# saidwivedi/TokenHMR

Hardware: NVIDIA H100
Metric: images/sec (256x192) at bs=64 per GPU, full TokenHMR forward (higher is better)
Workload: dtype f16 operands / f32 accumulate

## Files before the change

tokenhmr_b200/csrc/gemm_host.cuh:

```cuda
#pragma once
#include "common.cuh"

#include "gemm_wgmma.cuh"

namespace thmr {

struct GemmPlan {
  CUtensorMap tmA, tmB;
  GemmParams p;
  int bn;
  int grid;
  int cluster;
  int fp8;
  int epi;
};

struct GemmDesc {
  const __half* A; int lda; long long a_rows;
  const __half* B; int ldb;
  int M, N, K;
  const float* bias = nullptr;
  const float* resid = nullptr; int ldr = 0; int resid_mod = 0;
  int act = kActNone; int act32 = 0;
  float* out32 = nullptr; int ld32 = 0;
  __half* out16 = nullptr; int ld16 = 0;
  int taps = 1; int cin = 0; int tap_row0 = 0; int tap_stride = 0;
  int seq_pitch = 0, seq_lo = 0, seq_hi = 0;
  float alpha = 1.0f;
  long long* argmin_out = nullptr; const float* row_sq = nullptr; const float* col_sq = nullptr;
  int* screen_rows = nullptr; int* screen_count = nullptr; const float* screen_cmax2 = nullptr;
  float screen_rel = 0.f, screen_abs = 0.f; int screen_row0 = 0;
  const int* row_map = nullptr; const int* m_dev = nullptr; int m_dev_off = 0;
  int force_bn = 0;
  int force_epi = 0;
  unsigned long long* stamp = nullptr;
  int fp8 = 0;
  const float* a_scale = nullptr; int ld_as = 0;
  const float* w_scale = nullptr;
  uint8_t* out8 = nullptr; int ld8 = 0; float* out8_scale = nullptr; int ld8s = 0;
};

inline int pick_bn(int M, int N, int K, bool staged_epilogue, bool fast_epilogue, int force) {
  if (force) return force;
  const int sms = num_sms();
  const int tm = (M + kGemmBM - 1) / kGemmBM;
  const int num_kb = (K + kGemmBK - 1) / kGemmBK;
  int best = 256;
  double best_cost = -1;
  const int cands[4] = {256, 128, 64, 32};
  for (int i = 0; i < 4; ++i) {
    const int bn = cands[i];
    const long tiles = static_cast<long>(tm) * ((N + bn - 1) / bn);
    const long waves = (tiles + sms - 1) / sms;
    const double mma = 4.0 * bn;
    const double feed = (128.0 + bn) * 128.0 / 32.0;
    const double epilogue = !staged_epilogue                 ? 0.0
                            : fast_epilogue && bn >= 128      ? 5000.0 * bn / 128
                            : bn == 256                       ? 55000.0
                                                              : 7000.0 * bn / 128;
    const double cost = waves * (num_kb * ((mma > feed ? mma : feed) + 40.0) + epilogue);
    if (best_cost < 0 || cost < best_cost) { best_cost = cost; best = bn; }
  }
  return best;
}

inline int pick_bn_fp8(int M, int N, int K) {
  const int sms = num_sms();
  const int tm = (M + kGemmBM - 1) / kGemmBM;
  const int num_kb = (K + 127) / 128;
  int best = 128;
  double best_cost = -1;
  const int cands[2] = {128, 64};
  for (int i = 0; i < 2; ++i) {
    const int bn = cands[i];
    const long tiles = static_cast<long>(tm) * ((N + bn - 1) / bn);
    const long waves = (tiles + sms - 1) / sms;
    const double mma = 4.0 * bn;
    const double feed = (128.0 + bn) * 128.0 / 32.0;
    const double cost = waves * (num_kb * ((mma > feed ? mma : feed) + bn + 40.0) + 7000.0 * bn / 128);
    if (best_cost < 0 || cost < best_cost) { best_cost = cost; best = bn; }
  }
  return best;
}

inline int gemm_pick_epi(const GemmDesc& d, int bn, int cluster) {
  auto al16 = [](const void* q) { return (reinterpret_cast<uintptr_t>(q) & 15) == 0; };
  if ((bn != 128 && bn != 256) || cluster != 1 || d.argmin_out || d.resid_mod || d.seq_pitch || d.act32 || !al16(d.bias))
    return kEpiGeneral;
  if (d.out16 && !d.out32 && !d.resid && d.ld16 % 8 == 0 && al16(d.out16)) {
    if (d.act == kActNone) return d.bias ? kEpiBiasF16 : kEpiF16;
    if (d.act == kActGelu && d.bias) return kEpiBiasGeluF16;
  }
// ... 5 lines not shown

inline int make_tmap_2d_e4m3(CUtensorMap* out, const void* base, uint64_t rows, uint64_t cols, uint64_t ld,
                             uint32_t box_rows, uint32_t box_cols) {
  return make_tmap_2d(out, CU_TENSOR_MAP_DATA_TYPE_UINT8, 1, base, rows, cols, ld, box_rows, box_cols,
                      CU_TENSOR_MAP_SWIZZLE_128B);
}

inline int gemm_make_plan_fp8(const GemmDesc& d, GemmPlan* plan) {
  THMR_CHECK(d.M > 0 && d.N > 0 && d.K > 0 && d.K % 128 == 0, "gemm fp8: bad shape %dx%dx%d (K %% 128 != 0)", d.M, d.N,
             d.K);
  THMR_CHECK(d.out32 || d.out16 || d.out8, "gemm fp8: no output");
  THMR_CHECK(d.a_scale && d.w_scale, "gemm fp8: missing block scales");
  THMR_CHECK(!d.argmin_out && d.taps == 1 && !d.m_dev && !d.row_map, "gemm fp8: plain GEMMs only");
  const long m_pad = (d.M + kGemmBM - 1) / kGemmBM * kGemmBM;
  THMR_CHECK(d.ld_as >= m_pad && d.ld_as % 4 == 0 && (reinterpret_cast<uintptr_t>(d.a_scale) & 15) == 0,
             "gemm fp8: activation scales need a 16-byte aligned [K/128][>= %ld] layout (ld_as %d)", m_pad, d.ld_as);
  int bn = d.force_bn ? d.force_bn : d.out8 ? 128 : pick_bn_fp8(d.M, d.N, d.K);
  THMR_CHECK(bn == 64 || bn == 128, "gemm fp8: block_n %d (64 or 128)", bn);
  THMR_CHECK(!d.out8 || (bn == 128 && d.out8_scale && d.ld8s >= d.M && !d.resid && !d.act32 && !d.seq_pitch),
             "gemm fp8: e4m3 output needs block_n 128, its scale array and no residual / mask / act32");
  GemmParams& p = plan->p;
  memset(&p, 0, sizeof(p));
  p.M = d.M; p.N = d.N; p.K = d.K;
  p.out32 = d.out32; p.ld32 = d.ld32; p.out16 = d.out16; p.ld16 = d.ld16;
  p.bias = d.bias; p.resid = d.resid; p.ldr = d.ldr; p.resid_mod = d.resid_mod; p.act = d.act; p.act32 = d.act32;
  p.seq_pitch = d.seq_pitch; p.seq_lo = d.seq_lo; p.seq_hi = d.seq_hi;
  p.alpha = d.alpha;
  p.stamp = d.stamp;
  p.kblocks_per_tap = d.K / 128;
  p.a_scale = d.a_scale; p.ld_as = d.ld_as; p.w_scale = d.w_scale;
  p.out8 = d.out8; p.ld8 = d.ld8; p.out8_scale = d.out8_scale; p.ld8s = d.ld8s;
  THMR_TRY(make_tmap_2d_e4m3(&plan->tmA, d.A, d.a_rows, d.K, d.lda, kGemmBM, 128));
  THMR_TRY(make_tmap_2d_e4m3(&plan->tmB, d.B, d.N, d.K, d.ldb, bn, 128));
  THMR_CHECK(d.force_epi == 0 || d.force_epi == 1 + kEpiGeneral, "gemm fp8: general epilogue only");
  plan->bn = bn;
  plan->cluster = 1;
  plan->fp8 = 1;
  plan->epi = kEpiGeneral;
  const long tiles_m = (d.M + kGemmBM - 1) / kGemmBM;
  const long tiles = tiles_m * ((d.N + bn - 1) / bn);
  p.m_fast = (tiles_m > 1 && d.M < d.N) ? 1 : 0;
  const long slots = num_sms();
  plan->grid = static_cast<int>(tiles < slots ? tiles : slots);
  return THMR_OK;
}

inline int gemm_make_plan(const GemmDesc& d, GemmPlan* plan) {
  if (d.fp8) return gemm_make_plan_fp8(d, plan);
  THMR_CHECK(d.M > 0 && d.N > 0 && d.K > 0, "gemm: bad shape %dx%dx%d", d.M, d.N, d.K);
  THMR_CHECK(d.out32 || d.out16 || d.argmin_out, "gemm: no output");
  const int cluster = d.force_bn == 512 ? 2 : 1;
  THMR_CHECK(cluster == 1 || !d.argmin_out, "gemm: block_n 512 (CTA pair) does not support the arg-min modes");
  const bool fast_epi = gemm_pick_epi(d, 256, cluster) != kEpiGeneral;
  const int bn = cluster == 2 ? 256 : pick_bn(d.M, d.N, d.K, d.argmin_out == nullptr, fast_epi, d.force_bn);
  THMR_CHECK(bn == 32 || bn == 64 || bn == 128 || bn == 256, "gemm: bad block_n %d", bn);
  GemmParams& p = plan->p;
  memset(&p, 0, sizeof(p));
  p.M = d.M; p.N = d.N; p.K = d.K;
  p.out32 = d.out32; p.ld32 = d.ld32; p.out16 = d.out16; p.ld16 = d.ld16;
  p.bias = d.bias; p.resid = d.resid; p.ldr = d.ldr; p.resid_mod = d.resid_mod; p.act = d.act; p.act32 = d.act32;
  p.seq_pitch = d.seq_pitch; p.seq_lo = d.seq_lo; p.seq_hi = d.seq_hi;
  p.alpha = d.alpha; p.argmin_out = d.argmin_out; p.row_sq = d.row_sq; p.col_sq = d.col_sq;
  THMR_CHECK(!d.screen_rows || (d.argmin_out && d.screen_count && d.screen_cmax2),
             "gemm: screened arg-min needs its queue");
  THMR_CHECK((!d.m_dev && !d.row_map) || d.argmin_out, "gemm: device row count / row map are arg-min options");
  p.screen_rows = d.screen_rows; p.screen_count = d.screen_count; p.screen_cmax2 = d.screen_cmax2;
  p.screen_rel = d.screen_rel; p.screen_abs = d.screen_abs; p.screen_row0 = d.screen_row0;
  p.row_map = d.row_map; p.m_dev = d.m_dev; p.m_dev_off = d.m_dev_off;
  p.stamp = d.stamp;
  const int num_kb = (d.K + kGemmBK - 1) / kGemmBK;
  uint64_t a_cols = d.K;
  if (d.taps > 1) {
    THMR_CHECK(d.cin % kGemmBK == 0 && d.K == d.taps * d.cin, "gemm conv: cin %d taps %d K %d", d.cin, d.taps, d.K);
    p.kblocks_per_tap = d.cin / kGemmBK;
    p.tap_row0 = d.tap_row0; p.tap_stride = d.tap_stride;
    a_cols = d.cin;
  } else {
    p.kblocks_per_tap = num_kb;
  }
  THMR_TRY(make_tmap_2d_f16(&plan->tmA, d.A, d.a_rows, a_cols, d.lda, kGemmBM, kGemmBK, CU_TENSOR_MAP_SWIZZLE_128B));
  THMR_TRY(make_tmap_2d_f16(&plan->tmB, d.B, d.N, d.K, d.ldb, bn / cluster, kGemmBK, CU_TENSOR_MAP_SWIZZLE_128B));
  plan->bn = bn;
  plan->cluster = cluster;
  plan->fp8 = 0;
  plan->epi = gemm_pick_epi(d, bn, cluster);
  THMR_CHECK(d.force_epi == 0 || d.force_epi - 1 == kEpiGeneral || d.force_epi - 1 == plan->epi,
             "gemm: epilogue kind %d does not fit this GEMM (its kind is %d)", d.force_epi - 1, plan->epi);
  if (d.force_epi) plan->epi = d.force_epi - 1;
  const long tiles_m = (d.M + kGemmBM * cluster - 1) / (kGemmBM * cluster);
  const long tiles = d.argmin_out ? tiles_m : tiles_m * ((d.N + bn - 1) / bn);
  p.m_fast = (!d.argmin_out && tiles_m > 1 && d.M < d.N) ? 1 : 0;
  const long slots = num_sms() / cluster;
  plan->grid = cluster * static_cast<int>(tiles < slots ? tiles : slots);
  return THMR_OK;
}

template <int BN, int STAGES, int CLUSTER = 1, bool FP8 = false, int EPI = kEpiGeneral, bool TIMELINE = false>
inline int gemm_launch_t(const GemmPlan& plan, cudaStream_t stream) {
  using S = GemmSmem<BN, STAGES, FP8>;
  static_assert(S::kTotal <= 232448, "GEMM shared memory exceeds 227 KB");
  static bool configured = false;
  if (!configured) {
    THMR_CUDA(cudaFuncSetAttribute(gemm_f16_tn_kernel<BN, STAGES, CLUSTER, FP8, EPI, TIMELINE>, cudaFuncAttributeMaxDynamicSharedMemorySize,
                                   S::kTotal));
    configured = true;
  }
  cudaLaunchConfig_t cfg = {};
  cfg.gridDim = dim3(plan.grid);
  cfg.blockDim = dim3(kGemmThreads);
  cfg.dynamicSmemBytes = S::kTotal;
  cfg.stream = stream;
  cudaLaunchAttribute attr[1];
  attr[0].id = cudaLaunchAttributeClusterDimension;
  attr[0].val.clusterDim.x = CLUSTER;
  attr[0].val.clusterDim.y = 1;
  attr[0].val.clusterDim.z = 1;
  cfg.attrs = attr;
  cfg.numAttrs = 1;
  THMR_CUDA(cudaLaunchKernelEx(&cfg, gemm_f16_tn_kernel<BN, STAGES, CLUSTER, FP8, EPI, TIMELINE>, plan.tmA, plan.tmB, plan.p));
  return THMR_OK;
}

template <int BN, int STAGES, bool TIMELINE>
inline int gemm_launch_epi(const GemmPlan& plan, cudaStream_t stream) {
  switch (plan.epi) {
    case kEpiGeneral: return gemm_launch_t<BN, STAGES, 1, false, kEpiGeneral, TIMELINE>(plan, stream);
    case kEpiF16: return gemm_launch_t<BN, STAGES, 1, false, kEpiF16, TIMELINE>(plan, stream);
    case kEpiBiasF16: return gemm_launch_t<BN, STAGES, 1, false, kEpiBiasF16, TIMELINE>(plan, stream);
    case kEpiBiasGeluF16: return gemm_launch_t<BN, STAGES, 1, false, kEpiBiasGeluF16, TIMELINE>(plan, stream);
    case kEpiBiasResidF32: return gemm_launch_t<BN, STAGES, 1, false, kEpiBiasResidF32, TIMELINE>(plan, stream);
  }
  return fail(THMR_ERR_INVALID, "gemm: unsupported epilogue kind %d", plan.epi);
}

inline int gemm_launch_plain(const GemmPlan& plan, cudaStream_t stream) {
  if (plan.fp8) {
    if (plan.bn == 128) return gemm_launch_t<128, 5, 1, true>(plan, stream);
    if (plan.bn == 64) return gemm_launch_t<64, 7, 1, true>(plan, stream);
    return fail(THMR_ERR_INVALID, "gemm fp8: unsupported block_n %d", plan.bn);
  }
  if (plan.cluster == 2) return gemm_launch_t<256, 4, 2>(plan, stream);
  switch (plan.bn) {
    case 256: return gemm_launch_epi<256, 4, false>(plan, stream);
    case 128: return gemm_launch_epi<128, 6, false>(plan, stream);
    case 64: return gemm_launch_t<64, 8>(plan, stream);
    case 32: return gemm_launch_t<32, 8>(plan, stream);
  }
  return fail(THMR_ERR_INVALID, "gemm: unsupported block_n %d", plan.bn);
}

template <bool TIMELINE = false>
inline int gemm_launch(const GemmPlan& plan, cudaStream_t stream) {
// ... 13 lines not shown
```

tokenhmr_b200/csrc/gemm_wgmma.cuh:

```cuda
#pragma once
#include "common.cuh"
#include "ptx.cuh"

namespace thmr {

enum : int { kActNone = 0, kActGelu = 1, kActRelu = 2 };

enum : int { kEpiGeneral = 0, kEpiF16 = 1, kEpiBiasF16 = 2, kEpiBiasGeluF16 = 3, kEpiBiasResidF32 = 4 };

struct GemmParams {
  int M, N, K;
  float* out32;
  int ld32;
  __half* out16;
  int ld16;
  const float* bias;
  const float* resid;
  int ldr;
  int resid_mod;
  int act;
  int act32;
  int kblocks_per_tap;
  int tap_row0, tap_stride;
  int seq_pitch, seq_lo, seq_hi;
  float alpha;
  long long* argmin_out;
  const float* row_sq;
  const float* col_sq;
  int* screen_rows;
  int* screen_count;
  const float* screen_cmax2;
  float screen_rel, screen_abs;
  int screen_row0;
  const int* row_map;
  const int* m_dev;
  int m_dev_off;
  unsigned long long* stamp;
  int m_fast;
  const float* a_scale;
  int ld_as;
  const float* w_scale;
// ... 17 lines not shown
    m_blk = start;
    n_blk = 0;
  }
  __device__ bool valid() const { return m_stationary ? (m_blk < tiles_m) : (tile < num_tiles); }
  __device__ int m0(int bm) const { return (m_stationary ? m_blk : (m_fast ? tile % tiles_m : tile / tiles_n)) * bm; }
  __device__ int n0(int bn) const { return (m_stationary ? n_blk : (m_fast ? tile / tiles_m : tile % tiles_n)) * bn; }
  __device__ bool last_n() const { return n_blk == tiles_n - 1; }
  __device__ void next() {
    if (m_stationary) {
      if (++n_blk == tiles_n) { n_blk = 0; m_blk += stride; }
    } else {
      tile += stride;
    }
  }
};

constexpr int kGemmBM = 128;
constexpr int kGemmBK = 64;
constexpr int kGemmConsumerWarps = 8;
constexpr int kGemmThreads = 32 * kGemmConsumerWarps + 128;
constexpr int kWarpTma = kGemmConsumerWarps;

template <int BN>
constexpr int gemm_chunk() { return BN == 64 || BN == 128 ? 64 : 32; }

template <bool FP8>
constexpr int gemm_bk() { return FP8 ? 128 : kGemmBK; }

template <int BN, int STAGES, bool FP8 = false>
struct GemmSmem {
  static constexpr uint32_t kABytes = kGemmBM * kGemmBK * 2;
  static constexpr uint32_t kBBytes = BN * kGemmBK * 2;
  static constexpr uint32_t kStageBytes = kABytes + kBBytes;
  static constexpr uint32_t kScaleOffset = STAGES * kStageBytes;
  static constexpr uint32_t kScaleBytes = FP8 ? STAGES * kGemmBM * 4 : 0;
  static constexpr uint32_t kBarOffset = kScaleOffset + kScaleBytes;
  static constexpr uint32_t kEpiOffset = kBarOffset + 256;
  static constexpr uint32_t kEpiBytes = 2 * 64 * gemm_chunk<BN>() * 4;
  static constexpr uint32_t kRowScaleOffset = kEpiOffset + kEpiBytes;
  static constexpr uint32_t kRowScaleBytes = FP8 ? kGemmBM * 4 : 0;
  static constexpr uint32_t kTotal = kRowScaleOffset + kRowScaleBytes + 1024;
};

__device__ __forceinline__ float gelu_erf(float x) {
  const float a = fabsf(x) * 0.70710678118654752f;
  float p = fmaf(0.0000430638f, a, 0.0002765672f);
  p = fmaf(p, a, 0.0001520143f);
  p = fmaf(p, a, 0.0092705272f);
  p = fmaf(p, a, 0.0422820123f);
  p = fmaf(p, a, 0.0705230784f);
  p = fmaf(p, a, 1.0f);
  p *= p; p *= p; p *= p; p *= p;
  float r;
  asm("rcp.approx.ftz.f32 %0, %1;" : "=f"(r) : "f"(p));
  const float e = 1.0f - r;
  return fmaf(x, 0.5f, __fmul_rn(__fmul_rn(fabsf(x), 0.5f), e));
}

template <int BN>
__device__ __forceinline__ void wgmma_tile_k16(float (&acc)[BN / 2], uint64_t da, uint64_t db, uint32_t scale_d) {
  if constexpr (BN == 32) wgmma_m64n32k16(acc, da, db, scale_d);
  else if constexpr (BN == 64) wgmma_m64n64k16(acc, da, db, scale_d);
  else if constexpr (BN == 128) wgmma_m64n128k16(acc, da, db, scale_d);
  else wgmma_m64n256k16(acc, da, db, scale_d);
}

template <int BN>
__device__ __forceinline__ void wgmma_tile_k32_e4m3(float (&acc)[BN / 2], uint64_t da, uint64_t db, uint32_t scale_d) {
  if constexpr (BN == 64) wgmma_m64n64k32_e4m3(acc, da, db, scale_d);
  else wgmma_m64n128k32_e4m3(acc, da, db, scale_d);
}

// ... 132 lines not shown
          if (full && p.ld8 % 8 == 0 && (reinterpret_cast<uintptr_t>(p.out8) & 7) == 0) {
            *reinterpret_cast<uint2*>(o) = make_uint2(q[0] | (static_cast<uint32_t>(q[1]) << 16),
                                                      q[2] | (static_cast<uint32_t>(q[3]) << 16));
          } else {
#pragma unroll
            for (int e = 0; e < 8; ++e)
              if (col + e < p.N) o[e] = static_cast<uint8_t>(q[e >> 1] >> (8 * (e & 1)));
          }
        }
      }
      if (p.out16) {
        if (!p.act32 && !final_vals) {
#pragma unroll
          for (int e = 0; e < 8; ++e) v[e] = gemm_act(p.act, v[e]);
        }
        __half* o = p.out16 + static_cast<size_t>(row) * p.ld16 + col;
        if (full && vec16) {
          uint4 q;
          __half2* h2 = reinterpret_cast<__half2*>(&q);
#pragma unroll
          for (int e = 0; e < 4; ++e) h2[e] = __floats2half2_rn(v[2 * e], v[2 * e + 1]);
          *reinterpret_cast<uint4*>(o) = q;
        } else {
#pragma unroll
          for (int e = 0; e < 8; ++e)
            if (col + e < p.N) o[e] = __float2half_rn(v[e]);
        }
      }
    }
    named_barrier_sync(bar_id, 128);
  }
}

template <int EPI>
__device__ __forceinline__ void gemm_epilogue_kind_tail(const GemmParams& p, const float (&v)[8], int row, int col) {
#pragma unroll
  for (int e = 0; e < 8; ++e) {
    if (col + e >= p.N) break;
    float x = __fmul_rn(v[e], p.alpha);
    if constexpr (EPI != kEpiF16) x = __fadd_rn(x, __ldg(p.bias + col + e));
    if constexpr (EPI == kEpiBiasResidF32) {
      const size_t i = static_cast<size_t>(row) * p.ld32 + col + e;
      p.out32[i] = __fadd_rn(x, p.resid[static_cast<size_t>(row) * p.ldr + col + e]);
    } else {
      if constexpr (EPI == kEpiBiasGeluF16) x = gelu_erf(x);
      p.out16[static_cast<size_t>(row) * p.ld16 + col + e] = __float2half_rn(x);
    }
  }
}

template <int BN, int EPI>
__device__ __forceinline__ void gemm_epilogue_kind(const GemmParams& p, const float (&acc)[BN / 2], uint32_t stage,
                                                   int m0w, int n0, int M_eff, uint32_t bar_id) {
  constexpr bool kBias = EPI != kEpiF16;
  constexpr bool kResid = EPI == kEpiBiasResidF32;
  constexpr int CH = gemm_chunk<BN>();
  constexpr int OCT = CH / 8;
  constexpr int ITEMS = OCT / 2;
  const int lane = threadIdx.x & 31;
  const int w4 = (threadIdx.x >> 5) & 3;
  const int fr = w4 * 16 + (lane >> 2);
  const int fswz = (((lane >> 2) & 3) << 1) | ((lane >> 4) & 1);
  const int rswz = ((lane & 3) << 1) | ((lane >> 2) & 1);
#pragma unroll 1
  for (int c = 0; c < BN / CH; ++c) {
#pragma unroll
    for (int cc = 0; cc < BN / CH; ++cc)
      if (cc == c) gemm_stage_chunk<BN>(acc, cc, stage, fr, fswz, lane);
    named_barrier_sync(bar_id, 128);

    const int ccol = n0 + c * CH + 8 * (lane >> 3);
    float bias[ITEMS / 2][8];
    float res[ITEMS][8];
    if constexpr (kBias && !(kResid && ITEMS == 2)) {
#pragma unroll
      for (int ob = 0; ob < ITEMS / 2; ++ob) {
        const int col = ccol + 32 * ob;
        if (col + 8 <= p.N) {
          const float4 b0 = __ldg(reinterpret_cast<const float4*>(p.bias + col));
          const float4 b1 = __ldg(reinterpret_cast<const float4*>(p.bias + col + 4));
          bias[ob][0] = b0.x; bias[ob][1] = b0.y; bias[ob][2] = b0.z; bias[ob][3] = b0.w;
          bias[ob][4] = b1.x; bias[ob][5] = b1.y; bias[ob][6] = b1.z; bias[ob][7] = b1.w;
        }
      }
    }
    if constexpr (kResid) {
#pragma unroll
      for (int k = 0; k < ITEMS; ++k) {
        const int row = m0w + 8 * (w4 + 4 * (k & 1)) + (lane & 7);
        const int col = ccol + 32 * (k >> 1);
        if (row < M_eff && col + 8 <= p.N) {
          const float* r = p.resid + static_cast<size_t>(row) * p.ldr + col;
          const float4 x0 = *reinterpret_cast<const float4*>(r);
          const float4 x1 = *reinterpret_cast<const float4*>(r + 4);
          res[k][0] = x0.x; res[k][1] = x0.y; res[k][2] = x0.z; res[k][3] = x0.w;
          res[k][4] = x1.x; res[k][5] = x1.y; res[k][6] = x1.z; res[k][7] = x1.w;
        }
      }
    }
#pragma unroll
    for (int k = 0; k < ITEMS; ++k) {
      const int lr = 8 * (w4 + 4 * (k & 1)) + (lane & 7);
      const int oct = 4 * (k >> 1) + (lane >> 3);
      const int row = m0w + lr;
      const int col = ccol + 32 * (k >> 1);
      if (row >= M_eff || col >= p.N) continue;
      float v[8];
#pragma unroll
      for (int h = 0; h < 2; ++h) {
        const int u = 2 * oct + h;
        const float4 s = lds_f32x4(stage + 4 * (lr * CH + (((u & ~7) | ((u ^ rswz) & 7)) << 2)));
        v[4 * h] = s.x; v[4 * h + 1] = s.y; v[4 * h + 2] = s.z; v[4 * h + 3] = s.w;
      }
      if (col + 8 > p.N) {
        gemm_epilogue_kind_tail<EPI>(p, v, row, col);
        continue;
      }
      if constexpr (kResid && ITEMS == 2) {
        const float4 b0 = __ldg(reinterpret_cast<const float4*>(p.bias + col));
        const float4 b1 = __ldg(reinterpret_cast<const float4*>(p.bias + col + 4));
        bias[0][0] = b0.x; bias[0][1] = b0.y; bias[0][2] = b0.z; bias[0][3] = b0.w;
        bias[0][4] = b1.x; bias[0][5] = b1.y; bias[0][6] = b1.z; bias[0][7] = b1.w;
      }
#pragma unroll
      for (int e = 0; e < 8; ++e) {
        v[e] = __fmul_rn(v[e], p.alpha);
        if constexpr (kBias) v[e] = __fadd_rn(v[e], bias[k >> 1][e]);
        if constexpr (kResid) v[e] = __fadd_rn(v[e], res[k][e]);
        if constexpr (EPI == kEpiBiasGeluF16) v[e] = gelu_erf(v[e]);
      }
      if constexpr (kResid) {
        float4* o = reinterpret_cast<float4*>(p.out32 + static_cast<size_t>(row) * p.ld32 + col);
        o[0] = make_float4(v[0], v[1], v[2], v[3]);
        o[1] = make_float4(v[4], v[5], v[6], v[7]);
      } else {
        uint4 q;
        __half2* h2 = reinterpret_cast<__half2*>(&q);
#pragma unroll
        for (int e = 0; e < 4; ++e) h2[e] = __floats2half2_rn(v[2 * e], v[2 * e + 1]);
        *reinterpret_cast<uint4*>(p.out16 + static_cast<size_t>(row) * p.ld16 + col) = q;
      }
    }
    named_barrier_sync(bar_id, 128);
  }
}

template <int BN>
__device__ __forceinline__ void gemm_row_scales_e4m3(const GemmParams& p, float (&acc)[BN / 2], int m0, int n0,
                                                     int r0, int c0, int wg, int M_eff, uint32_t row_inv) {
#pragma unroll
  for (int i = 0; i < 2; ++i) {
    float amax = 0.f;
#pragma unroll
    for (int j = 0; j < BN / 8; ++j) {
#pragma unroll
      for (int c = 0; c < 2; ++c) {
        const int col = n0 + 8 * j + c0 + c;
        float v = acc[4 * j + 2 * i + c] * p.alpha;
        if (p.bias && col < p.N) v += __ldg(p.bias + col);
        v = gemm_act(p.act, v);
        acc[4 * j + 2 * i + c] = v;
        if (col < p.N) amax = fmaxf(amax, fabsf(v));
      }
    }
    amax = fmaxf(amax, __shfl_xor_sync(0xffffffffu, amax, 1));
    amax = fmaxf(amax, __shfl_xor_sync(0xffffffffu, amax, 2));
    const float s = e4m3_scale(amax);
    const int r = r0 + 8 * i;
    if ((threadIdx.x & 3) == 0) {
      sts_f32(row_inv + 4 * (r - wg * 64), 1.0f / s);
      if (m0 + r < M_eff) p.out8_scale[static_cast<size_t>(n0 / 128) * p.ld8s + m0 + r] = s;
    }
  }
}

template <int BN, int STAGES, int CLUSTER, bool FP8 = false, int EPI = kEpiGeneral, bool TIMELINE = false>
__global__ void __launch_bounds__(kGemmThreads, 1)
gemm_f16_tn_kernel(const __grid_constant__ CUtensorMap tmA, const __grid_constant__ CUtensorMap tmB, const GemmParams p) {
  using S = GemmSmem<BN, STAGES, FP8>;
  constexpr int BK = gemm_bk<FP8>();
  static_assert(BN == 32 || BN == 64 || BN == 128 || BN == 256, "BN must be a power of two in [32,256]");
  static_assert(CLUSTER == 1 || (CLUSTER == 2 && BN >= 128), "cluster pairs split B in two halves of >= 64 rows");
  static_assert(!FP8 || (CLUSTER == 1 && (BN == 64 || BN == 128)), "FP8: two accumulator sets fit at BN <= 128");
  static_assert(EPI == kEpiGeneral || (!FP8 && CLUSTER == 1 && BN >= 128), "epilogue kinds: fp16 BN 128 / 256 only");
  static_assert(!TIMELINE || (!FP8 && CLUSTER == 1), "timeline: fp16 single-CTA kernels only");

  extern __shared__ uint8_t smem_raw[];
  uint8_t* smem = reinterpret_cast<uint8_t*>((reinterpret_cast<uintptr_t>(smem_raw) + 1023) & ~uintptr_t(1023));
  uint64_t* full_bar = reinterpret_cast<uint64_t*>(smem + S::kBarOffset);
  uint64_t* empty_bar = full_bar + STAGES;

  const int warp = threadIdx.x >> 5;
  const int lane = threadIdx.x & 31;

  int M_eff = p.M;
  if (p.m_dev != nullptr) {
    const int m = __ldg(p.m_dev) - p.m_dev_off;
    M_eff = m < 0 ? 0 : (m < p.M ? m : p.M);
  }
  constexpr int kRows = kGemmBM * CLUSTER;
  const int tiles_m = (M_eff + kRows - 1) / kRows;
  const int tiles_n = (p.N + BN - 1) / BN;
  const int num_kb = (p.K + BK - 1) / BK;
  const bool m_stationary = p.argmin_out != nullptr;
  const int rank = CLUSTER == 2 ? static_cast<int>(cluster_ctarank()) : 0;
  const int tile0 = static_cast<int>(blockIdx.x) / CLUSTER, tile_step = static_cast<int>(gridDim.x) / CLUSTER;

  stamp_start(p.stamp);
  if (threadIdx.x == 0) {
    for (int s = 0; s < STAGES; ++s) {
      mbar_init(&full_bar[s], 1);
      mbar_init(&empty_bar[s], kGemmConsumerWarps * CLUSTER);
    }
    fence_mbar_init();
  }
  if (warp == kWarpTma && lane == 0) {
    tma_prefetch_desc(&tmA);
    tma_prefetch_desc(&tmB);
  }
  if constexpr (CLUSTER == 2) cluster_sync_all();
  else __syncthreads();

  if (warp >= kWarpTma) {
    asm volatile("setmaxnreg.dec.sync.aligned.u32 40;");
    if (warp == kWarpTma && lane == 0) {
      int stage = 0;
      uint32_t phase = 0;
      for (TileIter it(tiles_m, tiles_n, m_stationary, p.m_fast != 0, tile0, tile_step); it.valid(); it.next()) {
        const int m0 = it.m0(kRows) + rank * kGemmBM;
        const int n0 = it.n0(BN);
        for (int kb = 0; kb < num_kb; ++kb) {
          if constexpr (CLUSTER == 2) mbar_wait_cluster(&empty_bar[stage], phase ^ 1);
          else mbar_wait(&empty_bar[stage], phase ^ 1);
          uint8_t* sa = smem + stage * S::kStageBytes;
          uint8_t* sb = sa + S::kABytes;
          const int tap = kb / p.kblocks_per_tap;
          const int kk = kb - tap * p.kblocks_per_tap;
          mbar_arrive_expect_tx(&full_bar[stage], S::kStageBytes + (FP8 ? kGemmBM * 4 : 0));
          tma_load_2d(sa, &tmA, &full_bar[stage], kk * BK, m0 + p.tap_row0 + tap * p.tap_stride);
          if constexpr (CLUSTER == 2)
            tma_load_2d_mcast(sb + rank * (BN / 2) * 128, &tmB, &full_bar[stage], kb * BK, n0 + rank * (BN / 2), 3);
          else
            tma_load_2d(sb, &tmB, &full_bar[stage], kb * BK, n0);
          if constexpr (FP8)
            bulk_load_1d(smem + S::kScaleOffset + stage * kGemmBM * 4, p.a_scale + static_cast<size_t>(kb) * p.ld_as + m0,
                         kGemmBM * 4, &full_bar[stage]);
          if (++stage == STAGES) { stage = 0; phase ^= 1; }
        }
      }
    }
    if constexpr (CLUSTER == 2) cluster_sync_all();
    return;
  }

  asm volatile("setmaxnreg.inc.sync.aligned.u32 232;");
  const int wg = warp >> 2;
  const uint32_t smem_base = smem_u32(smem);
  const bool vec_r = p.resid && p.ldr % 4 == 0 && aligned16(p.resid);
  const bool vec32 = p.out32 && p.ld32 % 4 == 0 && aligned16(p.out32);
  const bool vec16 = p.out16 && p.ld16 % 8 == 0 && aligned16(p.out16);
  const uint32_t epi_stage = smem_base + S::kEpiOffset + wg * 64 * gemm_chunk<BN>() * 4;
  const bool screen = p.argmin_out != nullptr && p.screen_rows != nullptr;
  const float m2a = -2.0f * p.alpha;
  const int r0 = wg * 64 + (warp & 3) * 16 + (lane >> 2);
  const int c0 = 2 * (lane & 3);
  float best[2] = {INFINITY, INFINITY}, second[2] = {INFINITY, INFINITY};
  int best_idx[2] = {0, 0};
  int stage = 0;
  uint32_t phase = 0;
  float acc[BN / 2];
  float tile[FP8 ? BN / 2 : 1];

  auto release = [&](int s) {
    __syncwarp();
    if (lane == 0) {
      if constexpr (CLUSTER == 2) {
        mbar_arrive_cluster(&empty_bar[s], 0);
        mbar_arrive_cluster(&empty_bar[s], 1);
      } else {
        mbar_arrive(&empty_bar[s]);
      }
    }
  };
  auto stamp = [&](const TileIter& it, int k) {
    if (TIMELINE && p.timeline != nullptr && (threadIdx.x & 127) == 0) {
      const int slot = (it.tile - tile0) / tile_step;
      if (slot < p.timeline_slots)
        p.timeline[((static_cast<size_t>(blockIdx.x) * p.timeline_slots + slot) * 2 + wg) * 4 + k] = globaltimer();
    }
  };
  if (TIMELINE && p.timeline != nullptr && threadIdx.x == 0) p.timeline_sm[blockIdx.x] = static_cast<int>(smid());
  for (TileIter it(tiles_m, tiles_n, m_stationary, p.m_fast != 0, tile0, tile_step); it.valid(); it.next()) {
    const int m0 = it.m0(kRows) + rank * kGemmBM;
    const int n0 = it.n0(BN);
// ... 77 lines not shown
#pragma unroll
          for (int off = 1; off <= 2; off <<= 1) {
            const float ob = __shfl_xor_sync(0xffffffffu, best[i], off);
            const int oi = __shfl_xor_sync(0xffffffffu, best_idx[i], off);
            const float os = __shfl_xor_sync(0xffffffffu, second[i], off);
            second[i] = fminf(fminf(second[i], os), fmaxf(best[i], ob));
            if (ob < best[i] || (ob == best[i] && oi < best_idx[i])) { best[i] = ob; best_idx[i] = oi; }
          }
          const int row = m0 + r0 + 8 * i;
          const bool row_ok = row < M_eff;
          if ((lane & 3) == 0 && row_ok) p.argmin_out[p.row_map ? __ldg(p.row_map + row) : row] = best_idx[i];
          if (screen) {
            const float x2 = row_ok ? __ldg(p.row_sq + row) : 0.f;
            const float tau = p.screen_rel * sqrtf(x2 * cm2) + p.screen_abs * (x2 + cm2) + 1e-12f;
            const bool redo = (lane & 3) == 0 && row_ok && !(second[i] - best[i] > tau);
            const unsigned mask = __ballot_sync(0xffffffffu, redo);
            if (mask != 0u) {
              const int leader = __ffs(mask) - 1;
              int base = 0;
              if (lane == leader) base = atomicAdd(p.screen_count, __popc(mask));
              base = __shfl_sync(0xffffffffu, base, leader);
              if (redo) p.screen_rows[base + __popc(mask & ((1u << lane) - 1u))] = p.screen_row0 + row;
            }
          }
          best[i] = INFINITY;
          second[i] = INFINITY;
          best_idx[i] = 0;
        }
      }
    } else if constexpr (FP8) {
      const uint32_t row_inv = smem_base + S::kRowScaleOffset + wg * 64 * 4;
      if (p.out8) gemm_row_scales_e4m3<BN>(p, acc, m0, n0, r0, c0, wg, M_eff, row_inv);
      gemm_epilogue_rows<BN, true>(p, acc, epi_stage, m0 + wg * 64, n0, M_eff, 1 + wg, vec_r, vec32, vec16, row_inv);
    } else if constexpr (EPI != kEpiGeneral) {
      gemm_epilogue_kind<BN, EPI>(p, acc, epi_stage, m0 + wg * 64, n0, M_eff, 1 + wg);
    } else {
      gemm_epilogue_rows<BN>(p, acc, epi_stage, m0 + wg * 64, n0, M_eff, 1 + wg, vec_r, vec32, vec16);
    }
    if constexpr (TIMELINE) stamp(it, 3);
  }
  if constexpr (CLUSTER == 2) cluster_sync_all();
}

}
```

tokenhmr_b200/csrc/ptx.cuh:

```cuda
#pragma once
#include <cuda.h>
#include <cuda_fp16.h>
#include <cuda_runtime.h>
#include <stdint.h>

namespace thmr {

__device__ unsigned int g_pipeline_timeout = 0;
constexpr uint32_t kSpinLimit = 1u << 24;

__device__ __forceinline__ uint32_t smem_u32(const void* p) {
  return static_cast<uint32_t>(__cvta_generic_to_shared(p));
}

__device__ __forceinline__ void sts_f32x2(uint32_t a, float x, float y) {
  asm volatile("st.shared.v2.f32 [%0], {%1, %2};" ::"r"(a), "f"(x), "f"(y));
}
__device__ __forceinline__ float4 lds_f32x4(uint32_t a) {
  float4 v;
  asm volatile("ld.shared.v4.f32 {%0, %1, %2, %3}, [%4];" : "=f"(v.x), "=f"(v.y), "=f"(v.z), "=f"(v.w) : "r"(a));
  return v;
}
__device__ __forceinline__ void sts_f32(uint32_t a, float x) { asm volatile("st.shared.f32 [%0], %1;" ::"r"(a), "f"(x)); }
__device__ __forceinline__ float lds_f32(uint32_t a) {
  float v;
  asm volatile("ld.shared.f32 %0, [%1];" : "=f"(v) : "r"(a));
  return v;
}
__device__ __forceinline__ void named_barrier_sync(uint32_t id, uint32_t threads) {
  asm volatile("bar.sync %0, %1;" ::"r"(id), "r"(threads) : "memory");
}

__device__ __forceinline__ unsigned long long globaltimer() {
  unsigned long long t;
  asm volatile("mov.u64 %0, %%globaltimer;" : "=l"(t));
  return t;
}
__device__ __forceinline__ uint32_t smid() {
  uint32_t s;
  asm volatile("mov.u32 %0, %%smid;" : "=r"(s));
  return s;
}

__device__ __forceinline__ uint32_t lane_id() {
  uint32_t l;
  asm volatile("mov.u32 %0, %%laneid;" : "=r"(l));
  return l;
}

__device__ __forceinline__ void mbar_init(uint64_t* bar, uint32_t count) {
  asm volatile("mbarrier.init.shared::cta.b64 [%0], %1;" ::"r"(smem_u32(bar)), "r"(count) : "memory");
}
__device__ __forceinline__ void fence_mbar_init() {
  asm volatile("fence.mbarrier_init.release.cluster;" ::: "memory");
}
__device__ __forceinline__ void fence_proxy_async_smem() {
// ... 57 lines not shown
        "selp.u32 %0, 1, 0, P;\n\t"
        "}\n"
        : "=r"(ok)
        : "r"(smem_u32(bar)), "r"(parity)
        : "memory");
    if (ok) return true;
  }
  atomicExch(&g_pipeline_timeout, 1u);
  return false;
}

__device__ __forceinline__ void tma_prefetch_desc(const CUtensorMap* m) {
  asm volatile("prefetch.tensormap [%0];" ::"l"(reinterpret_cast<uint64_t>(m)) : "memory");
}
__device__ __forceinline__ void tma_load_2d(void* smem_dst, const CUtensorMap* m, uint64_t* bar, int32_t c0,
                                            int32_t c1) {
  asm volatile(
      "cp.async.bulk.tensor.2d.shared::cluster.global.mbarrier::complete_tx::bytes"
      " [%0], [%1, {%3, %4}], [%2];"
      :
      : "r"(smem_u32(smem_dst)), "l"(reinterpret_cast<uint64_t>(m)), "r"(smem_u32(bar)), "r"(c0), "r"(c1)
      : "memory");
}
__device__ __forceinline__ void tma_load_2d_mcast(void* smem_dst, const CUtensorMap* m, uint64_t* bar, int32_t c0,
                                                  int32_t c1, uint16_t cta_mask) {
  asm volatile(
      "cp.async.bulk.tensor.2d.shared::cluster.global.mbarrier::complete_tx::bytes.multicast::cluster"
      " [%0], [%1, {%3, %4}], [%2], %5;"
      :
      : "r"(smem_u32(smem_dst)), "l"(reinterpret_cast<uint64_t>(m)), "r"(smem_u32(bar)), "r"(c0), "r"(c1),
        "h"(cta_mask)
      : "memory");
}
__device__ __forceinline__ void tma_store_2d(const CUtensorMap* m, const void* smem_src, int32_t c0, int32_t c1) {
  asm volatile("cp.async.bulk.tensor.2d.global.shared::cta.bulk_group [%0, {%2, %3}], [%1];"
               :
               : "l"(reinterpret_cast<uint64_t>(m)), "r"(smem_u32(smem_src)), "r"(c0), "r"(c1)
               : "memory");
}
__device__ __forceinline__ void tma_store_commit() { asm volatile("cp.async.bulk.commit_group;" ::: "memory"); }
template <int N>
__device__ __forceinline__ void tma_store_wait_read() {
  asm volatile("cp.async.bulk.wait_group.read %0;" ::"n"(N) : "memory");
}
template <int N>
__device__ __forceinline__ void tma_store_wait() {
  asm volatile("cp.async.bulk.wait_group %0;" ::"n"(N) : "memory");
}

__device__ __forceinline__ uint64_t make_wgmma_desc_sw128(uint32_t saddr) {
  uint64_t d = 0;
  d |= static_cast<uint64_t>((saddr >> 4) & 0x3FFF);
  d |= static_cast<uint64_t>(1) << 16;
  d |= static_cast<uint64_t>(1024 >> 4) << 32;
  d |= static_cast<uint64_t>(1) << 62;
  return d;
}
__device__ __forceinline__ void wgmma_fence() { asm volatile("wgmma.fence.sync.aligned;" ::: "memory"); }
__device__ __forceinline__ void wgmma_commit() { asm volatile("wgmma.commit_group.sync.aligned;" ::: "memory"); }
template <int N>
__device__ __forceinline__ void wgmma_wait() {
  asm volatile("wgmma.wait_group.sync.aligned %0;" ::"n"(N) : "memory");
}
template <int N>
__device__ __forceinline__ void wgmma_fence_operand(float (&d)[N]) {
#pragma unroll
  for (int i = 0; i < N; ++i) asm volatile("" : "+f"(d[i])::"memory");
}

__device__ __forceinline__ void wgmma_m64n32k16(float (&d)[16], uint64_t da, uint64_t db, uint32_t scale_d) {
// ... 65 lines not shown
```

Baseline: 1690.

## Store fp16 GEMM epilogues through swizzled shared memory with TMA bulk stores

The fp16 epilogue kinds (plain, bias, bias+GELU) now convert accumulators to half, write them into a 128B-swizzled shared-memory staging block and issue asynchronous TMA 2D stores, instead of staging fp32 and having threads write global memory. A third tensor map for the output is built on the host and passed to the kernel. The residual fp32 epilogue is split into its own specialised function, and the block-N cost model now weights TMA-store and residual epilogues differently. The shared-memory layout grows each warpgroup's epilogue block to 16 KB, and the kernel waits for outstanding stores before exiting. The aim is to cut epilogue time and let stores overlap with the next tile's main loop.

```diff
diff --git a/tokenhmr_b200/csrc/gemm_host.cuh b/tokenhmr_b200/csrc/gemm_host.cuh
--- a/tokenhmr_b200/csrc/gemm_host.cuh
+++ b/tokenhmr_b200/csrc/gemm_host.cuh
@@ -7,6 +7,7 @@
 
 struct GemmPlan {
   CUtensorMap tmA, tmB;
+  CUtensorMap tmC;
   GemmParams p;
   int bn;
   int grid;
@@ -40,7 +41,7 @@
   uint8_t* out8 = nullptr; int ld8 = 0; float* out8_scale = nullptr; int ld8s = 0;
 };
 
-inline int pick_bn(int M, int N, int K, bool staged_epilogue, bool fast_epilogue, int force) {
+inline int pick_bn(int M, int N, int K, bool staged_epilogue, int epi_kind, int force) {
   if (force) return force;
   const int sms = num_sms();
   const int tm = (M + kGemmBM - 1) / kGemmBM;
@@ -54,10 +55,11 @@
     const long waves = (tiles + sms - 1) / sms;
     const double mma = 4.0 * bn;
     const double feed = (128.0 + bn) * 128.0 / 32.0;
-    const double epilogue = !staged_epilogue                 ? 0.0
-                            : fast_epilogue && bn >= 128      ? 5000.0 * bn / 128
-                            : bn == 256                       ? 55000.0
-                                                              : 7000.0 * bn / 128;
+    const double epilogue = !staged_epilogue                                 ? 0.0
+                            : bn >= 128 && gemm_epi_tma_store(epi_kind)       ? 2500.0 * bn / 128
+                            : bn >= 128 && epi_kind == kEpiBiasResidF32       ? 12000.0 * bn / 128
+                            : bn == 256                                       ? 55000.0
+                                                                              : 7000.0 * bn / 128;
     const double cost = waves * (num_kb * ((mma > feed ? mma : feed) + 40.0) + epilogue);
     if (best_cost < 0 || cost < best_cost) { best_cost = cost; best = bn; }
   }
@@ -129,6 +131,7 @@
   p.out8 = d.out8; p.ld8 = d.ld8; p.out8_scale = d.out8_scale; p.ld8s = d.ld8s;
   THMR_TRY(make_tmap_2d_e4m3(&plan->tmA, d.A, d.a_rows, d.K, d.lda, kGemmBM, 128));
   THMR_TRY(make_tmap_2d_e4m3(&plan->tmB, d.B, d.N, d.K, d.ldb, bn, 128));
+  memset(&plan->tmC, 0, sizeof(plan->tmC));
   THMR_CHECK(d.force_epi == 0 || d.force_epi == 1 + kEpiGeneral, "gemm fp8: general epilogue only");
   plan->bn = bn;
   plan->cluster = 1;
@@ -148,8 +151,8 @@
   THMR_CHECK(d.out32 || d.out16 || d.argmin_out, "gemm: no output");
   const int cluster = d.force_bn == 512 ? 2 : 1;
   THMR_CHECK(cluster == 1 || !d.argmin_out, "gemm: block_n 512 (CTA pair) does not support the arg-min modes");
-  const bool fast_epi = gemm_pick_epi(d, 256, cluster) != kEpiGeneral;
-  const int bn = cluster == 2 ? 256 : pick_bn(d.M, d.N, d.K, d.argmin_out == nullptr, fast_epi, d.force_bn);
+  const int kind = gemm_pick_epi(d, 256, cluster);
+  const int bn = cluster == 2 ? 256 : pick_bn(d.M, d.N, d.K, d.argmin_out == nullptr, kind, d.force_bn);
   THMR_CHECK(bn == 32 || bn == 64 || bn == 128 || bn == 256, "gemm: bad block_n %d", bn);
   GemmParams& p = plan->p;
   memset(&p, 0, sizeof(p));
@@ -184,6 +187,9 @@
   THMR_CHECK(d.force_epi == 0 || d.force_epi - 1 == kEpiGeneral || d.force_epi - 1 == plan->epi,
              "gemm: epilogue kind %d does not fit this GEMM (its kind is %d)", d.force_epi - 1, plan->epi);
   if (d.force_epi) plan->epi = d.force_epi - 1;
+  memset(&plan->tmC, 0, sizeof(plan->tmC));
+  if (gemm_epi_tma_store(plan->epi))
+    THMR_TRY(make_tmap_2d_f16(&plan->tmC, d.out16, d.M, d.N, d.ld16, 64, 64, CU_TENSOR_MAP_SWIZZLE_128B));
   const long tiles_m = (d.M + kGemmBM * cluster - 1) / (kGemmBM * cluster);
   const long tiles = d.argmin_out ? tiles_m : tiles_m * ((d.N + bn - 1) / bn);
   p.m_fast = (!d.argmin_out && tiles_m > 1 && d.M < d.N) ? 1 : 0;
@@ -214,7 +220,8 @@
   attr[0].val.clusterDim.z = 1;
   cfg.attrs = attr;
   cfg.numAttrs = 1;
-  THMR_CUDA(cudaLaunchKernelEx(&cfg, gemm_f16_tn_kernel<BN, STAGES, CLUSTER, FP8, EPI, TIMELINE>, plan.tmA, plan.tmB, plan.p));
+  THMR_CUDA(cudaLaunchKernelEx(&cfg, gemm_f16_tn_kernel<BN, STAGES, CLUSTER, FP8, EPI, TIMELINE>, plan.tmA, plan.tmB,
+                               plan.tmC, plan.p));
   return THMR_OK;
 }
 
diff --git a/tokenhmr_b200/csrc/gemm_wgmma.cuh b/tokenhmr_b200/csrc/gemm_wgmma.cuh
--- a/tokenhmr_b200/csrc/gemm_wgmma.cuh
+++ b/tokenhmr_b200/csrc/gemm_wgmma.cuh
@@ -7,6 +7,8 @@
 enum : int { kActNone = 0, kActGelu = 1, kActRelu = 2 };
 
 enum : int { kEpiGeneral = 0, kEpiF16 = 1, kEpiBiasF16 = 2, kEpiBiasGeluF16 = 3, kEpiBiasResidF32 = 4 };
+
+constexpr bool gemm_epi_tma_store(int epi) { return epi == kEpiF16 || epi == kEpiBiasF16 || epi == kEpiBiasGeluF16; }
 
 struct GemmParams {
   int M, N, K;
@@ -90,12 +92,14 @@
   static constexpr uint32_t kABytes = kGemmBM * kGemmBK * 2;
   static constexpr uint32_t kBBytes = BN * kGemmBK * 2;
   static constexpr uint32_t kStageBytes = kABytes + kBBytes;
-  static constexpr uint32_t kScaleOffset = STAGES * kStageBytes;
+  static constexpr uint32_t kEpiOffset = STAGES * kStageBytes;
+  static constexpr uint32_t kEpiWgBytes = 64 * 128 * 2;
+  static_assert(64 * gemm_chunk<BN>() * 4 <= kEpiWgBytes, "fp32 staging chunk exceeds the warpgroup's block");
+  static constexpr uint32_t kEpiBytes = 2 * kEpiWgBytes;
+  static constexpr uint32_t kScaleOffset = kEpiOffset + kEpiBytes;
   static constexpr uint32_t kScaleBytes = FP8 ? STAGES * kGemmBM * 4 : 0;
   static constexpr uint32_t kBarOffset = kScaleOffset + kScaleBytes;
-  static constexpr uint32_t kEpiOffset = kBarOffset + 256;
-  static constexpr uint32_t kEpiBytes = 2 * 64 * gemm_chunk<BN>() * 4;
-  static constexpr uint32_t kRowScaleOffset = kEpiOffset + kEpiBytes;
+  static constexpr uint32_t kRowScaleOffset = kBarOffset + 256;
   static constexpr uint32_t kRowScaleBytes = FP8 ? kGemmBM * 4 : 0;
   static constexpr uint32_t kTotal = kRowScaleOffset + kRowScaleBytes + 1024;
 };
@@ -294,28 +298,19 @@
   }
 }
 
-template <int EPI>
-__device__ __forceinline__ void gemm_epilogue_kind_tail(const GemmParams& p, const float (&v)[8], int row, int col) {
+__device__ __forceinline__ void gemm_epilogue_resid_tail(const GemmParams& p, const float (&v)[8], int row, int col) {
 #pragma unroll
   for (int e = 0; e < 8; ++e) {
     if (col + e >= p.N) break;
-    float x = __fmul_rn(v[e], p.alpha);
-    if constexpr (EPI != kEpiF16) x = __fadd_rn(x, __ldg(p.bias + col + e));
-    if constexpr (EPI == kEpiBiasResidF32) {
-      const size_t i = static_cast<size_t>(row) * p.ld32 + col + e;
-      p.out32[i] = __fadd_rn(x, p.resid[static_cast<size_t>(row) * p.ldr + col + e]);
-    } else {
-      if constexpr (EPI == kEpiBiasGeluF16) x = gelu_erf(x);
-      p.out16[static_cast<size_t>(row) * p.ld16 + col + e] = __float2half_rn(x);
-    }
-  }
-}
-
-template <int BN, int EPI>
-__device__ __forceinline__ void gemm_epilogue_kind(const GemmParams& p, const float (&acc)[BN / 2], uint32_t stage,
-                                                   int m0w, int n0, int M_eff, uint32_t bar_id) {
-  constexpr bool kBias = EPI != kEpiF16;
-  constexpr bool kResid = EPI == kEpiBiasResidF32;
+    const float x = __fadd_rn(__fmul_rn(v[e], p.alpha), __ldg(p.bias + col + e));
+    const float r = p.resid[static_cast<size_t>(row) * p.ldr + col + e];
+    p.out32[static_cast<size_t>(row) * p.ld32 + col + e] = __fadd_rn(x, r);
+  }
+}
+
+template <int BN>
+__device__ __forceinline__ void gemm_epilogue_resid(const GemmParams& p, const float (&acc)[BN / 2], uint32_t stage,
+                                                    int m0w, int n0, int M_eff, uint32_t bar_id) {
   constexpr int CH = gemm_chunk<BN>();
   constexpr int OCT = CH / 8;
   constexpr int ITEMS = OCT / 2;
@@ -334,7 +329,7 @@
     const int ccol = n0 + c * CH + 8 * (lane >> 3);
     float bias[ITEMS / 2][8];
     float res[ITEMS][8];
-    if constexpr (kBias && !(kResid && ITEMS == 2)) {
+    if constexpr (ITEMS != 2) {
 #pragma unroll
       for (int ob = 0; ob < ITEMS / 2; ++ob) {
         const int col = ccol + 32 * ob;
@@ -346,18 +341,16 @@
         }
       }
     }
-    if constexpr (kResid) {
-#pragma unroll
-      for (int k = 0; k < ITEMS; ++k) {
-        const int row = m0w + 8 * (w4 + 4 * (k & 1)) + (lane & 7);
-        const int col = ccol + 32 * (k >> 1);
-        if (row < M_eff && col + 8 <= p.N) {
-          const float* r = p.resid + static_cast<size_t>(row) * p.ldr + col;
-          const float4 x0 = *reinterpret_cast<const float4*>(r);
-          const float4 x1 = *reinterpret_cast<const float4*>(r + 4);
-          res[k][0] = x0.x; res[k][1] = x0.y; res[k][2] = x0.z; res[k][3] = x0.w;
-          res[k][4] = x1.x; res[k][5] = x1.y; res[k][6] = x1.z; res[k][7] = x1.w;
-        }
+#pragma unroll
+    for (int k = 0; k < ITEMS; ++k) {
+      const int row = m0w + 8 * (w4 + 4 * (k & 1)) + (lane & 7);
+      const int col = ccol + 32 * (k >> 1);
+      if (row < M_eff && col + 8 <= p.N) {
+        const float* r = p.resid + static_cast<size_t>(row) * p.ldr + col;
+        const float4 x0 = *reinterpret_cast<const float4*>(r);
+        const float4 x1 = *reinterpret_cast<const float4*>(r + 4);
+        res[k][0] = x0.x; res[k][1] = x0.y; res[k][2] = x0.z; res[k][3] = x0.w;
+        res[k][4] = x1.x; res[k][5] = x1.y; res[k][6] = x1.z; res[k][7] = x1.w;
       }
     }
 #pragma unroll
@@ -375,35 +368,71 @@
         v[4 * h] = s.x; v[4 * h + 1] = s.y; v[4 * h + 2] = s.z; v[4 * h + 3] = s.w;
       }
       if (col + 8 > p.N) {
-        gemm_epilogue_kind_tail<EPI>(p, v, row, col);
+        gemm_epilogue_resid_tail(p, v, row, col);
         continue;
       }
-      if constexpr (kResid && ITEMS == 2) {
+      if constexpr (ITEMS == 2) {
         const float4 b0 = __ldg(reinterpret_cast<const float4*>(p.bias + col));
         const float4 b1 = __ldg(reinterpret_cast<const float4*>(p.bias + col + 4));
         bias[0][0] = b0.x; bias[0][1] = b0.y; bias[0][2] = b0.z; bias[0][3] = b0.w;
         bias[0][4] = b1.x; bias[0][5] = b1.y; bias[0][6] = b1.z; bias[0][7] = b1.w;
       }
 #pragma unroll
-      for (int e = 0; e < 8; ++e) {
-        v[e] = __fmul_rn(v[e], p.alpha);
-        if constexpr (kBias) v[e] = __fadd_rn(v[e], bias[k >> 1][e]);
-        if constexpr (kResid) v[e] = __fadd_rn(v[e], res[k][e]);
-        if constexpr (EPI == kEpiBiasGeluF16) v[e] = gelu_erf(v[e]);
-      }
-      if constexpr (kResid) {
-        float4* o = reinterpret_cast<float4*>(p.out32 + static_cast<size_t>(row) * p.ld32 + col);
-        o[0] = make_float4(v[0], v[1], v[2], v[3]);
-        o[1] = make_float4(v[4], v[5], v[6], v[7]);
-      } else {
-        uint4 q;
-        __half2* h2 = reinterpret_cast<__half2*>(&q);
-#pragma unroll
-        for (int e = 0; e < 4; ++e) h2[e] = __floats2half2_rn(v[2 * e], v[2 * e + 1]);
-        *reinterpret_cast<uint4*>(p.out16 + static_cast<size_t>(row) * p.ld16 + col) = q;
-      }
+      for (int e = 0; e < 8; ++e)
+        v[e] = __fadd_rn(__fadd_rn(__fmul_rn(v[e], p.alpha), bias[k >> 1][e]), res[k][e]);
+      float4* o = reinterpret_cast<float4*>(p.out32 + static_cast<size_t>(row) * p.ld32 + col);
+      o[0] = make_float4(v[0], v[1], v[2], v[3]);
+      o[1] = make_float4(v[4], v[5], v[6], v[7]);
     }
     named_barrier_sync(bar_id, 128);
+  }
+}
+
+template <int BN, int EPI>
+__device__ __forceinline__ void gemm_epilogue_f16_tma(const GemmParams& p, const float (&acc)[BN / 2],
+                                                      const CUtensorMap* tm, uint32_t stage, int m0w, int n0,
+                                                      int M_eff, uint32_t bar_id) {
+  static_assert(gemm_epi_tma_store(EPI) && BN % 128 == 0, "fp16 TMA-store kinds, 128-column passes");
+  const int lane = threadIdx.x & 31;
+  const bool issuer = (threadIdx.x & 127) == 0;
+  const int fr = ((threadIdx.x >> 5) & 3) * 16 + (lane >> 2);
+  const int c0 = 2 * (lane & 3);
+  const int swz = lane >> 2;
+#pragma unroll
+  for (int q = 0; q < BN / 128; ++q) {
+    const int nq = n0 + 128 * q;
+    if (nq >= p.N) break;
+    if (issuer) tma_store_wait_read<0>();
+    named_barrier_sync(bar_id, 128);
+#pragma unroll
+    for (int j = 0; j < 16; ++j) {
+      const int col = nq + 8 * j + c0;
+      float b[2] = {0.f, 0.f};
+      if constexpr (EPI != kEpiF16) {
+        b[0] = __ldg(p.bias + min(col, p.N - 1));
+        b[1] = __ldg(p.bias + min(col + 1, p.N - 1));
+      }
+#pragma unroll
+      for (int i = 0; i < 2; ++i) {
+        float v[2];
+#pragma unroll
+        for (int c = 0; c < 2; ++c) {
+          v[c] = __fmul_rn(acc[64 * q + 4 * j + 2 * i + c], p.alpha);
+          if constexpr (EPI != kEpiF16) v[c] = __fadd_rn(v[c], b[c]);
+          if constexpr (EPI == kEpiBiasGeluF16) v[c] = gelu_erf(v[c]);
+        }
+        const __half2 h = __floats2half2_rn(v[0], v[1]);
+        sts_u32(stage + (j >> 3) * 8192 + (fr + 8 * i) * 128 + (((j & 7) ^ swz) << 4) + 2 * c0,
+                *reinterpret_cast<const uint32_t*>(&h));
+      }
+    }
+    fence_proxy_async_smem();
+    named_barrier_sync(bar_id, 128);
+    if (issuer && m0w < M_eff) {
+      tma_store_2d(tm, stage, nq, m0w);
+      if (nq + 64 < p.N) tma_store_2d(tm, stage + 8192, nq + 64, m0w);
+      tma_store_commit();
+    }
   }
 }
 
@@ -438,7 +467,8 @@
 
 template <int BN, int STAGES, int CLUSTER, bool FP8 = false, int EPI = kEpiGeneral, bool TIMELINE = false>
 __global__ void __launch_bounds__(kGemmThreads, 1)
-gemm_f16_tn_kernel(const __grid_constant__ CUtensorMap tmA, const __grid_constant__ CUtensorMap tmB, const GemmParams p) {
+gemm_f16_tn_kernel(const __grid_constant__ CUtensorMap tmA, const __grid_constant__ CUtensorMap tmB,
+                   const __grid_constant__ CUtensorMap tmC, const GemmParams p) {
   using S = GemmSmem<BN, STAGES, FP8>;
   constexpr int BK = gemm_bk<FP8>();
   static_assert(BN == 32 || BN == 64 || BN == 128 || BN == 256, "BN must be a power of two in [32,256]");
@@ -479,6 +509,7 @@
   if (warp == kWarpTma && lane == 0) {
     tma_prefetch_desc(&tmA);
     tma_prefetch_desc(&tmB);
+    if constexpr (gemm_epi_tma_store(EPI)) tma_prefetch_desc(&tmC);
   }
   if constexpr (CLUSTER == 2) cluster_sync_all();
   else __syncthreads();
@@ -521,7 +552,7 @@
   const bool vec_r = p.resid && p.ldr % 4 == 0 && aligned16(p.resid);
   const bool vec32 = p.out32 && p.ld32 % 4 == 0 && aligned16(p.out32);
   const bool vec16 = p.out16 && p.ld16 % 8 == 0 && aligned16(p.out16);
-  const uint32_t epi_stage = smem_base + S::kEpiOffset + wg * 64 * gemm_chunk<BN>() * 4;
+  const uint32_t epi_stage = smem_base + S::kEpiOffset + wg * S::kEpiWgBytes;
   const bool screen = p.argmin_out != nullptr && p.screen_rows != nullptr;
   const float m2a = -2.0f * p.alpha;
   const int r0 = wg * 64 + (warp & 3) * 16 + (lane >> 2);
@@ -665,13 +696,17 @@
       const uint32_t row_inv = smem_base + S::kRowScaleOffset + wg * 64 * 4;
       if (p.out8) gemm_row_scales_e4m3<BN>(p, acc, m0, n0, r0, c0, wg, M_eff, row_inv);
       gemm_epilogue_rows<BN, true>(p, acc, epi_stage, m0 + wg * 64, n0, M_eff, 1 + wg, vec_r, vec32, vec16, row_inv);
+    } else if constexpr (EPI == kEpiBiasResidF32) {
+      gemm_epilogue_resid<BN>(p, acc, epi_stage, m0 + wg * 64, n0, M_eff, 1 + wg);
     } else if constexpr (EPI != kEpiGeneral) {
-      gemm_epilogue_kind<BN, EPI>(p, acc, epi_stage, m0 + wg * 64, n0, M_eff, 1 + wg);
+      gemm_epilogue_f16_tma<BN, EPI>(p, acc, &tmC, epi_stage, m0 + wg * 64, n0, M_eff, 1 + wg);
     } else {
       gemm_epilogue_rows<BN>(p, acc, epi_stage, m0 + wg * 64, n0, M_eff, 1 + wg, vec_r, vec32, vec16);
     }
     if constexpr (TIMELINE) stamp(it, 3);
   }
+  if constexpr (gemm_epi_tma_store(EPI))
+    if ((threadIdx.x & 127) == 0) tma_store_wait<0>();
   if constexpr (CLUSTER == 2) cluster_sync_all();
 }
 
diff --git a/tokenhmr_b200/csrc/ptx.cuh b/tokenhmr_b200/csrc/ptx.cuh
--- a/tokenhmr_b200/csrc/ptx.cuh
+++ b/tokenhmr_b200/csrc/ptx.cuh
@@ -22,6 +22,7 @@
   return v;
 }
 __device__ __forceinline__ void sts_f32(uint32_t a, float x) { asm volatile("st.shared.f32 [%0], %1;" ::"r"(a), "f"(x)); }
+__device__ __forceinline__ void sts_u32(uint32_t a, uint32_t x) { asm volatile("st.shared.b32 [%0], %1;" ::"r"(a), "r"(x)); }
 __device__ __forceinline__ float lds_f32(uint32_t a) {
   float v;
   asm volatile("ld.shared.f32 %0, [%1];" : "=f"(v) : "r"(a));
@@ -145,10 +146,10 @@
         "h"(cta_mask)
       : "memory");
 }
-__device__ __forceinline__ void tma_store_2d(const CUtensorMap* m, const void* smem_src, int32_t c0, int32_t c1) {
+__device__ __forceinline__ void tma_store_2d(const CUtensorMap* m, uint32_t smem_src, int32_t c0, int32_t c1) {
   asm volatile("cp.async.bulk.tensor.2d.global.shared::cta.bulk_group [%0, {%2, %3}], [%1];"
                :
-               : "l"(reinterpret_cast<uint64_t>(m)), "r"(smem_u32(smem_src)), "r"(c0), "r"(c1)
+               : "l"(reinterpret_cast<uint64_t>(m)), "r"(smem_src), "r"(c0), "r"(c1)
                : "memory");
 }
 __device__ __forceinline__ void tma_store_commit() { asm volatile("cp.async.bulk.commit_group;" ::: "memory"); }
```

New measurement: 1803, median of 6. 1.07x the previous value.
